# alibaba/animate-anything

Measured on AMD Instinct MI355X. Metric: UNet3D denoising steps/sec @16fx512x512 bs=1, higher is better.
Workload: dtype fp16; 1 GPU; animate_anything_512_v1.02 UNet3D (1413M params, seeded random init), 16 frames x 512x512, pipeline bs=1 per GPU (CFG batch 2, 17 frames inside), DPM-Solver++ step, hipGraph=on; clips_per_gpu=1, clips=1, parallelism=clip-sharded x1, collective=none

## Files before the change

### animate_anything_amd/_lib.py

```python
from __future__ import annotations

import ctypes as C
import os

import torch

AA_F16, AA_BF16, AA_F32 = 0, 1, 2
AA_ACT_NONE, AA_ACT_SILU, AA_ACT_GELU, AA_ACT_QUICK_GELU = 0, 1, 2, 3


class AaConvGemm(C.Structure):
    _fields_ = [
        ("a0", C.c_void_p), ("a1", C.c_void_p), ("w", C.c_void_p), ("bias", C.c_void_p),
        ("rowvec", C.c_void_p), ("residual", C.c_void_p), ("out", C.c_void_p),
        ("c0", C.c_int32), ("c1", C.c_int32),
        ("n_img", C.c_int32), ("h_in", C.c_int32), ("w_in", C.c_int32), ("h_virt", C.c_int32),
        ("w_virt", C.c_int32), ("h_out", C.c_int32), ("w_out", C.c_int32),
        ("kh", C.c_int32), ("kw", C.c_int32), ("stride", C.c_int32), ("pad_h", C.c_int32), ("pad_w", C.c_int32),
        ("n_out", C.c_int32), ("n_pad", C.c_int32), ("k_pad", C.c_int32),
        ("rowvec_div", C.c_int32), ("ldo", C.c_int32), ("ldr", C.c_int32),
        ("act", C.c_int32), ("geglu", C.c_int32), ("bias_per_row", C.c_int32),
        ("dtype", C.c_int32), ("out_dtype", C.c_int32), ("out_scale", C.c_float), ("workspace", C.c_void_p), ("workspace_bytes", C.c_int64), ("k_order", C.c_int32), ("debug", C.c_int32), ("tile", C.c_int32), ("k_splits", C.c_int32), ("rowvec_ld", C.c_int32), ("acc_scale", C.c_float),
        ("out_sy", C.c_int32), ("out_sx", C.c_int32), ("out_oy", C.c_int32), ("out_ox", C.c_int32),
        ("ln_stats", C.c_void_p), ("ln_cols", C.c_void_p), ("ln_parts", C.c_int32), ("ln_eps", C.c_float),
# ... 145 lines not shown

class AaFreeU(C.Structure):
    _fields_ = [
        ("hidden", C.c_void_p), ("hidden_out", C.c_void_p), ("skip", C.c_void_p), ("skip_out", C.c_void_p), ("trig", C.c_void_p),
        ("images", C.c_int32), ("h", C.c_int32), ("w", C.c_int32), ("c_hidden", C.c_int32), ("c_skip", C.c_int32),
        ("hidden_ld", C.c_int32), ("hidden_out_ld", C.c_int32), ("skip_ld", C.c_int32), ("skip_out_ld", C.c_int32),
        ("b", C.c_float), ("s", C.c_float), ("dtype", C.c_int32),
    ]


class AaCfgRescale(C.Structure):
    _fields_ = [
        ("tokens", C.c_void_p), ("out", C.c_void_p), ("factor", C.c_void_p),
        ("clips", C.c_int32), ("channels", C.c_int32), ("frames", C.c_int32), ("hw", C.c_int32), ("ld", C.c_int32), ("out_ld", C.c_int32),
        ("guidance", C.c_float), ("rescale", C.c_float), ("dtype", C.c_int32),
    ]


AA_WINDOW_MAX = 64


class AaWindow(C.Structure):
    _fields_ = [
        ("window_frames", C.c_int32), ("frame", C.c_int32 * AA_WINDOW_MAX), ("weight", C.c_float * AA_WINDOW_MAX),
        ("first", C.c_int32 * AA_WINDOW_MAX), ("last", C.c_int32 * AA_WINDOW_MAX),
    ]


class AaWindowGather(C.Structure):
    _fields_ = [
        ("src", C.c_void_p), ("dst", C.c_void_p),
        ("clips", C.c_int32), ("channels", C.c_int32), ("total_frames", C.c_int32), ("hw", C.c_int32),
        ("window", AaWindow),
    ]


class AaWindowMerge(C.Structure):
    _fields_ = [
        ("tokens", C.c_void_p), ("acc", C.c_void_p), ("merged", C.c_void_p),
        ("clips", C.c_int32), ("channels", C.c_int32), ("total_frames", C.c_int32), ("hw", C.c_int32), ("ld", C.c_int32), ("out_ld", C.c_int32),
        ("guidance_on", C.c_int32), ("guidance", C.c_float), ("dtype", C.c_int32),
        ("window", AaWindow),
    ]


class AaFreeInit(C.Structure):
    _fields_ = [
        ("x", C.c_void_p), ("n0", C.c_void_p), ("z", C.c_void_p), ("out", C.c_void_p), ("mask", C.c_void_p), ("twiddle", C.c_void_p),
        ("volumes", C.c_int32), ("frames", C.c_int32), ("h", C.c_int32), ("w", C.c_int32),
        ("a", C.c_float), ("s", C.c_float),
    ]


_I, _I32, _I64, _F, _V, _Z, _P = C.c_int, C.c_int32, C.c_int64, C.c_float, C.c_void_p, C.c_size_t, C.POINTER


def _launch(desc):
    return _I, [_P(desc), _V]


PROTOTYPES = {
    "aa_version": (_I, []),
    "aa_last_error": (C.c_char_p, []),
    "aa_conv_gemm_workspace": (_Z, [_P(AaConvGemm)]),
    "aa_conv_gemm": _launch(AaConvGemm),
    "aa_conv_gemm_group": (_I, [_P(_P(AaConvGemm)), _I32, _V]),
    "aa_conv_gemm_group_ok": (_I, [_P(_P(AaConvGemm)), _I32, _I32]),
    "aa_conv_gemm_launch_count": (_I, [_P(AaConvGemm)]),
    "aa_conv_gemm_tickets": (_I, [_P(AaConvGemm)]),
    "aa_conv_gemm_reduce_launches": (_I, [_P(AaConvGemm)]),
    "aa_conv_gemm_row_stats_parts": (_I, [_P(AaConvGemm)]),
    "aa_conv_gemm_row_coef_ok": (_I, [_P(AaConvGemm)]),
    "aa_ln_finalize": (_I, [_V, _I32, _V, _I64, _I32, _F, _V]),
    "aa_conv_gemm_tile_info": (_I, [_I, _P(_I32)]),
    "aa_conv_gemm_tile_flags": (_I, [_I]),
    "aa_conv_gemm_tile_ok": (_I, [_P(AaConvGemm), _I]),
    "aa_set_tile_override": (None, [_I]),
    "aa_groupnorm_workspace": (_Z, [_P(AaGroupNorm)]),
    "aa_set_groupnorm_two_pass": (None, [_I]),
    "aa_groupnorm_plan": (_I, [_P(AaGroupNorm), _P(_I32)]),
    "aa_groupnorm": (_I, [_P(AaGroupNorm), _V, _Z, _V]),
    "aa_groupnorm_coef": (_I, [_P(AaGroupNorm), _V, _Z, _V, _V]),
    "aa_layernorm": (_I, [_V, _V, _V, _V, _I64, _I32, _F, _I32, _V]),
    "aa_attention": _launch(AaAttention),
    "aa_seq_self_attention_ok": (_I, [_P(AaSeqSelfAttn)]),
    "aa_seq_self_attention": _launch(AaSeqSelfAttn),
    "aa_ff_fused_ok": (_I, [_P(AaFFFused)]),
    "aa_ff_fused": _launch(AaFFFused),
    "aa_linear_rows_ok": (_I, [_P(AaLinearRows)]),
    "aa_linear_rows": _launch(AaLinearRows),
    "aa_quant_rows_fp8": _launch(AaQuantRowsFp8),
    "aa_linear_fp8": _launch(AaLinearFp8),
    "aa_softmax_rows": (_I, [_V, _V, _I64, _I32, _I32, _I32, _I32, _V]),
    "aa_cfg_dpm_step": _launch(AaDpmStep),
    "aa_timestep_embedding": (_I, [_V, _V, _I32, _I32, _I32, _V]),
    "aa_pack_latents": _launch(AaPackLatents),
    "aa_cfg_dpm_step_tokens": _launch(AaDpmStepTok),
    "aa_blend": _launch(AaBlend),
    "aa_pack_frames": _launch(AaPackFrames),
    "aa_cfg_euler_step_tokens": _launch(AaEulerStepTok),
    "aa_cfg_ddim_step_tokens": _launch(AaDdimStepTok),
    "aa_cfg_unipc_step_tokens": _launch(AaUnipcStepTok),
    "aa_freeu_tokens": _launch(AaFreeU),
    "aa_cfg_rescale_workspace": (_Z, [_P(AaCfgRescale)]),
    "aa_cfg_rescale_tokens": (_I, [_P(AaCfgRescale), _V, _Z, _V]),
    "aa_window_gather_latents": _launch(AaWindowGather),
    "aa_window_merge_tokens": _launch(AaWindowMerge),
    "aa_freeinit_workspace": (_Z, [_P(AaFreeInit)]),
    "aa_freeinit_mix": (_I, [_P(AaFreeInit), _V, _Z, _V]),
}
SYMBOLS = tuple(PROTOTYPES)

DEFAULT_PATH = os.path.join(os.path.dirname(os.path.abspath(__file__)), "libaa_mi355.so")


def bind(path: str) -> C.CDLL:
    if not os.path.exists(path):
        raise RuntimeError(f"{path} is missing: build it with `python -m animate_anything_amd.build` "
                           "(hipcc --offload-arch=gfx950); this package has no fallback backend")
    lib = C.CDLL(path)
    for name, (restype, argtypes) in PROTOTYPES.items():
        if not hasattr(lib, name):
            raise RuntimeError(f"{path} does not export {name}")
        fn = getattr(lib, name)
        fn.restype, fn.argtypes = restype, argtypes
    return lib


_lib = None
_host_pointers_ok = False


def get() -> C.CDLL:
    global _lib
    if _lib is None:
        _lib = bind(os.environ.get("AA_LIBRARY") or DEFAULT_PATH)
    return _lib


def host_pointers_ok() -> bool:
    return _host_pointers_ok


class use_library:

    def __init__(self, lib, host_pointers=False):
        self.lib, self.host = lib, host_pointers

    def __enter__(self):
        global _lib, _host_pointers_ok
        self.prev = (_lib, _host_pointers_ok)
        _lib, _host_pointers_ok = self.lib, self.host
        return self.lib

    def __exit__(self, *a):
        global _lib, _host_pointers_ok
        _lib, _host_pointers_ok = self.prev
```

### animate_anything_amd/build.py

```python
import os
import subprocess

PKG = os.path.dirname(os.path.abspath(__file__))
ROOT = os.path.dirname(PKG)
CSRC = os.path.join(PKG, "csrc")
LIB = os.path.join(PKG, "libaa_mi355.so")


def _deps():
    deps = [os.path.join(ROOT, "include", "aa_mi355.h")]
    for d, _, fs in os.walk(CSRC):
        deps += [os.path.join(d, f) for f in fs if f.endswith((".h", ".hip"))]
    return deps


def source_id():
    import hashlib
    h = hashlib.sha256()
    for d in sorted(_deps()):
        h.update(os.path.relpath(d, ROOT).encode())
        h.update(open(d, "rb").read())
    return h.hexdigest()[:16]


PROBE_LIB = os.path.join(PKG, "libaa_mi355_probe.so")
TU_GROUPS = 8


def build(force=False, verbose=False, probe=False, ablate=0, variant=None):
    LIB = PROBE_LIB if probe else globals()["LIB"]
    if ablate:
        LIB = os.path.join(PKG, f"libaa_mi355_abl{ablate}.so")
    if variant:
        LIB = os.path.join(PKG, f"libaa_mi355_{variant[0]}.so")
    if not force and os.path.exists(LIB) and all(os.path.getmtime(LIB) >= os.path.getmtime(d) for d in _deps()):
        return LIB
    hipcc = os.environ.get("HIPCC", "/opt/rocm/bin/hipcc")
    flags = ["--offload-arch=gfx950", "-O3", "-std=c++17", "-fPIC", "-ffast-math", f"-DAA_TU_GROUPS={TU_GROUPS}",
             "-I", os.path.join(CSRC, "kernels", "device"), "-I", os.path.join(CSRC, "kernels"), "-I", CSRC,
             "-I", os.path.join(ROOT, "include")]
    if probe:
        flags.insert(0, "-DAA_PHASE_PROBE")
    if ablate:
        flags.insert(0, f"-DAA_X_ABLATE={int(ablate)}")
    if variant:
        flags = list(variant[1]) + flags
    if verbose:
        flags.insert(0, "-Rpass-analysis=kernel-resource-usage")
    obj_dir = os.path.join(PKG, "build", os.path.basename(LIB)[:-3])
    os.makedirs(obj_dir, exist_ok=True)
    jobs = [([os.path.join(CSRC, "aa_api.hip")], os.path.join(obj_dir, "aa_api.o"))]
    jobs += [([f"-DAA_TU_GROUP={g}", os.path.join(CSRC, "aa_tiles.hip")], os.path.join(obj_dir, f"aa_tiles_{g}.o")) for g in range(TU_GROUPS)]

    import hashlib
    api_only = {"attention.h", "seq_attention.h", "norm.h", "glue.h", "freeu.h", "cfg_rescale.h", "window.h", "freeinit.h", "ff_fused.h", "linear_rows.h", "linear_fp8.h"}

    def dep_hash(job):
        src, _ = job
        h = hashlib.sha256(repr((flags, [x for x in src if x.startswith("-D")])).encode())
        tiles = any("aa_tiles.hip" in x for x in src)
        for d in sorted(_deps()):
            if tiles and (os.path.basename(d) in api_only or d.endswith("aa_api.hip")):
                continue
            if not tiles and d.endswith("aa_tiles.hip"):
                continue
            h.update(d.encode())
            h.update(open(d, "rb").read())
        return h.hexdigest()

    def compile_one(job):
        src, obj = job
        key, stamp = dep_hash(job), obj + ".dephash"
        if not force and os.path.exists(obj) and os.path.exists(stamp) and open(stamp).read() == key:
            return obj
        subprocess.check_call([hipcc] + flags + ["-c"] + src + ["-o", obj])
        with open(stamp, "w") as f:
            f.write(key)
        return obj

    from concurrent.futures import ThreadPoolExecutor
    with ThreadPoolExecutor(max_workers=max(1, min(len(jobs), os.cpu_count() or 1))) as pool:
        objs = list(pool.map(compile_one, jobs))
    subprocess.check_call([hipcc, "--offload-arch=gfx950", "-shared", "-fPIC"] + objs + ["-o", LIB])
    import shutil
    have_tools = shutil.which(os.path.join(LLVM_TOOLS, "llvm-objdump")) and shutil.which(os.path.join(LLVM_TOOLS, "llvm-readelf"))
    if not ablate and os.environ.get("AA_BUILD_AUDIT", "1") != "0" and not have_tools:
        import json
        with open(LIB[:-3] + ".buildinfo.json", "w") as f:
            json.dump({"flags": flags, "audit": "skipped: llvm-objdump / llvm-readelf not found under " + LLVM_TOOLS}, f, indent=1)
    elif not ablate and os.environ.get("AA_BUILD_AUDIT", "1") != "0":
        problems = audit_x_kernels(LIB)
        info = {"hipcc": subprocess.run([hipcc, "--version"], capture_output=True, text=True).stdout.strip().split("\n"),
                "flags": flags, "audit": "ok" if not problems else problems}
        import json
        with open(LIB[:-3] + ".buildinfo.json", "w") as f:
            json.dump(info, f, indent=1)
        if problems:
            os.replace(LIB, LIB + ".rejected")
            raise RuntimeError("libaa_mi355.so: the code-object audit of the hand-scheduled kernels failed (library moved to "
                               + LIB + ".rejected):\n  " + "\n  ".join(str(p_) for p_ in problems[:8]))
    return LIB


LLVM_TOOLS = "/opt/rocm/lib/llvm/bin"


def device_code_objects(lib_path, out_dir):
    import struct
# ... 146 lines not shown
```

### animate_anything_amd/csrc/aa_api_impl.h

```cpp
#pragma once
#include <stdarg.h>
#include <stdio.h>
#include <stdlib.h>
#include <string.h>
#include "aa_mi355.h"
#include "kernels/conv_gemm.h"
#include "kernels/conv_gemm_dma.h"
#include "kernels/conv_slab.h"
#include "kernels/conv_gemm_x.h"
#include "kernels/norm.h"
#include "kernels/attention.h"
#include "kernels/seq_attention.h"
#include "kernels/ff_fused.h"
#include "kernels/linear_rows.h"
#include "kernels/linear_fp8.h"
#include "kernels/glue.h"
#include "kernels/freeu.h"
#include "kernels/cfg_rescale.h"
#include "kernels/window.h"
#include "kernels/freeinit.h"

namespace aa {

static thread_local char g_err[512] = "";

static int fail(int code, const char* fmt, ...) {
    va_list ap;
    va_start(ap, fmt);
    vsnprintf(g_err, sizeof(g_err), fmt, ap);
    va_end(ap);
    return code;
}

static int finish(const char* what) {
    const char* e = AA_POST_LAUNCH();
    if (e) return fail(AA_E_HIP, "%s: %s", what, e);
    return AA_OK;
}

static bool aligned_to(const void* p, uintptr_t bytes) { return (reinterpret_cast<uintptr_t>(p) & (bytes - 1)) == 0; }
static bool aligned16(const void* p) { return aligned_to(p, 16); }

template <typename T> struct DType16 { using type = T; };
template <typename F>
static bool with_dtype16(int dtype, F&& f) {
    if (dtype == AA_F16) { f(DType16<f16_t>{}); return true; }
    if (dtype == AA_BF16) { f(DType16<bf16_t>{}); return true; }
    return false;
}

template <typename D>
static bool step_tok_geometry_ok(const D* d, int ld) {
    return d->clips > 0 && d->channels > 0 && d->frames > 0 && d->hw > 0 && ld >= d->channels && d->next_t_count >= 0 && d->next_t_count <= 256;
}

template <typename D>
static dim3 step_tok_grid(const D* d) {
    const int64_t blocks = ((int64_t)d->clips * d->channels * d->frames * d->hw + 255) / 256;
    return dim3((unsigned)(blocks > 2048 ? 2048 : blocks));
}

struct CgCfg { int bm, bn, wm, wn, bk, stages, per_cu; float rate; int slab = 0; int x = 0; int sched = 0; };
constexpr int cg_dp(int dp3, int dp0, int dp1) { return (dp3 | dp0 << 4 | dp1 << 8) << 6; }
static const CgCfg kCgCfgs[] = {
    {128, 64, 2, 2, 64, 2, 3, 0.78f},
    {128, 128, 2, 2, 64, 2, 2, 0.90f},
    {192, 256, 3, 2, 64, 2, 1, 1.05f},
    {256, 256, 4, 2, 64, 2, 1, 1.10f},
    {256, 320, 4, 2, 64, 2, 1, 1.10f},
    {192, 320, 3, 2, 64, 2, 1, 1.05f},
    {256, 320, 4, 2, 32, 4, 1, 1.15f},
    {256, 256, 4, 2, 32, 4, 1, 1.15f},
    {128, 128, 2, 2, 32, 4, 2, 0.95f},
// ... 1222 lines not shown
    const dim3 grid((unsigned)((d->hw + WIN_THREADS - 1) / WIN_THREADS), (unsigned)d->window.window_frames, (unsigned)d->clips), block(WIN_THREADS);
    with_dtype16(d->dtype, [&](auto t) {
        using T = typename decltype(t)::type;
        if (vec) AA_LAUNCH((window_merge_kernel<T, true>), grid, block, 0, stream, *d);
        else AA_LAUNCH((window_merge_kernel<T, false>), grid, block, 0, stream, *d);
    });
    return finish("window_merge_tokens");
}

static bool freeinit_geometry_ok(const AaFreeInit* d) {
    if (d->volumes < 1 || d->frames < 1 || d->h < 1 || d->w < 1 || d->frames > aa::FI_MAX || d->h > aa::FI_MAX || d->w > aa::FI_MAX) return false;
    return (int64_t)d->volumes * d->frames * d->h * d->w < ((int64_t)1 << 31);
}

size_t aa_freeinit_workspace(const AaFreeInit* d) {
    if (!d || !freeinit_geometry_ok(d)) return 0;
    return (size_t)d->volumes * d->frames * d->h * d->w * 2 * sizeof(float);
}

int aa_freeinit_mix(const AaFreeInit* d, void* workspace, size_t workspace_bytes, void* stream) {
    using namespace aa;
    if (!d || !d->x || !d->n0 || !d->z || !d->out || !d->mask || !d->twiddle) return fail(AA_E_SHAPE, "freeinit_mix: null operand");
    if (!freeinit_geometry_ok(d))
        return fail(AA_E_SHAPE, "freeinit_mix: bad geometry (volumes %d, frames %d, h %d, w %d; every axis 1 .. %d)", d->volumes, d->frames, d->h,
                    d->w, FI_MAX);
    if (!finite_f32(&d->a) || !finite_f32(&d->s)) return fail(AA_E_SHAPE, "freeinit_mix: a and s must be finite");
    const size_t need = aa_freeinit_workspace(d);
    if (!workspace || workspace_bytes < need) return fail(AA_E_WORKSPACE, "freeinit_mix: workspace %zu < %zu bytes", workspace_bytes, need);
    if (!aligned_to(d->x, 4) || !aligned_to(d->n0, 4) || !aligned_to(d->z, 4) || !aligned_to(d->out, 4) || !aligned_to(d->mask, 4) ||
        !aligned_to(d->twiddle, 8) || !aligned_to(workspace, 8))
        return fail(AA_E_ALIGN, "freeinit_mix: x / n0 / z / out / mask must be 4-byte, the table and the workspace 8-byte aligned");
    const int64_t vol = (int64_t)d->frames * d->h * d->w, n = vol * d->volumes;
    const Span out = {d->out, n * 4}, ws = {workspace, (int64_t)need};
    const Span in[5] = {{d->x, n * 4}, {d->n0, n * 4}, {d->z, n * 4}, {d->mask, vol * 4}, {d->twiddle, (int64_t)(d->frames + d->h + d->w) * 8}};
    if (spans_overlap(out, in[0]) && d->out != d->x) return fail(AA_E_SHAPE, "freeinit_mix: out may be x itself or a separate buffer, not overlap it");
    for (int i = 1; i < 5; ++i)
        if (spans_overlap(out, in[i])) return fail(AA_E_SHAPE, "freeinit_mix: out must not overlap n0, z, the mask or the table");
    if (spans_overlap(out, ws)) return fail(AA_E_SHAPE, "freeinit_mix: the workspace must not overlap out");
    for (int i = 0; i < 5; ++i)
        if (spans_overlap(ws, in[i])) return fail(AA_E_SHAPE, "freeinit_mix: the workspace must not overlap an operand");
    f32x2* spec = (f32x2*)workspace;
    const f32x2* tw = (const f32x2*)d->twiddle;
    const dim3 block(FI_THREADS), rows((unsigned)fi_row_groups(*d));
    AA_LAUNCH(freeinit_rows_fwd_kernel<>, rows, block, FI_ROWS_FWD_LDS, stream, *d, spec);
    AA_LAUNCH((freeinit_axis_kernel<false>), dim3((unsigned)fi_axis_groups((int64_t)d->volumes * d->frames, d->w)), block, FI_AXIS_LDS, stream, spec,
              tw + fi_tw_h(*d), d->h, d->w);
    AA_LAUNCH(freeinit_frames_kernel<>, dim3((unsigned)fi_axis_groups(d->volumes, (int64_t)d->h * d->w)), block, FI_FRAMES_LDS, stream, *d, spec);
    AA_LAUNCH((freeinit_axis_kernel<true>), dim3((unsigned)fi_axis_groups((int64_t)d->volumes * d->frames, d->w)), block, FI_AXIS_LDS, stream, spec,
              tw + fi_tw_h(*d), d->h, d->w);
    AA_LAUNCH(freeinit_rows_inv_kernel<>, rows, block, FI_ROWS_INV_LDS, stream, *d, (const f32x2*)spec);
    return finish("freeinit_mix");
}

}
#endif
```

### animate_anything_amd/ops.py

```python
from __future__ import annotations

import ctypes as C
import math
import os
from dataclasses import dataclass
from typing import Optional

import torch

from . import _lib
from ._lib import (AA_ACT_GELU, AA_ACT_NONE, AA_ACT_QUICK_GELU, AA_ACT_SILU, AA_BF16, AA_F16, AA_F32, AaAttention, AaAttnOperand,
                   AaBlend, AaConvGemm, AaFFFused, AaLinearRows, AaLinearFp8, AaQuantRowsFp8, AaDdimStepTok, AaDpmStep, AaDpmStepTok, AaEulerStepTok, AaGroupNorm, AaPackFrames, AaPackLatents, AaSeqSelfAttn, AaUnipcStepTok, AaFreeU, AaCfgRescale, AaWindow, AaWindowGather, AaWindowMerge, AaFreeInit)

_DT = {torch.float16: AA_F16, torch.bfloat16: AA_BF16, torch.float32: AA_F32}

TRACE = None

AUTOTUNE = True
LAST_STAMPS = None
GN_PLANS = None
MAX_OPERAND_BYTES = 1 << 31
FORCE_TILE = -1
ATTN_FLAGS = int(os.environ.get("AA_ATTN_FLAGS", "0"))
if ATTN_FLAGS & ~13:
    raise RuntimeError(f"AA_ATTN_FLAGS={ATTN_FLAGS}: only bits 0 (value 1), 2 (value 4) and 3 (value 8) exist")
LN_FINALIZE_LAUNCH = os.environ.get("AA_LN_RAW", "0") != "1"
TILE_PICKER = None
PRODUCER_COEF = os.environ.get("AA_PRODUCER_COEF", "1") == "1"
LN_RAW_ANY_PARTS = False
K_SPLITS = 0
USE_TICKETS = os.environ.get("AA_TICKETS", "0") == "1"
DEBUG_ABLATE = int(os.environ.get("AA_DEBUG_ABLATE", "0"))
class _TileTable:

    def __init__(self):
        self._rows = None

    def _load(self):
        if self._rows is None:
            lib, rows, info = _lib.get(), [], (C.c_int32 * 7)()
            while lib.aa_conv_gemm_tile_info(len(rows), info) == 0:
                rows.append(tuple(info) + (int(lib.aa_conv_gemm_tile_flags(len(rows))),))
            self._rows = rows
        return self._rows

    def __iter__(self):
        return iter([(r[0], r[1], r[4], r[5]) for r in self._load()])

    def __len__(self):
        return len(self._load())

    def __getitem__(self, i):
        r = self._load()[i]
        return (r[0], r[1], r[4], r[5])

    def wave_cols(self, i):
        return self._load()[i][3]

    def per_cu(self, i):
        return self._load()[i][6]

    def flags(self, i):
        return self._load()[i][7]


# ... 631 lines not shown
def groupnorm(x0: torch.Tensor, gamma: torch.Tensor, beta: torch.Tensor, n_groups_img: int,
              tokens_per_group: int, num_groups: int = 32, eps: float = 1e-5, silu: bool = False,
              x1: Optional[torch.Tensor] = None, out: Optional[torch.Tensor] = None) -> torch.Tensor:
    lib = _lib.get()
    _check(x0, x1, gamma, beta, out)
    c0 = x0.shape[-1]
    c1 = 0 if x1 is None else x1.shape[-1]
    y = torch.empty(n_groups_img * tokens_per_group, c0 + c1, dtype=x0.dtype, device=x0.device) if out is None else out
    d = AaGroupNorm()
    d.x0, d.x1, d.gamma, d.beta, d.y = _ptr(x0), _ptr(x1), _ptr(gamma), _ptr(beta), _ptr(y)
    d.c0, d.c1 = c0, c1
    d.n_groups_img, d.tokens_per_group, d.num_groups = n_groups_img, tokens_per_group, num_groups
    d.silu, d.dtype, d.eps = int(silu), _DT[x0.dtype], eps
    nbytes = lib.aa_groupnorm_workspace(C.byref(d))
    ws = torch.empty(max(nbytes // 4, 1), dtype=torch.float32, device=x0.device)
    two_pass = False
    if AUTOTUNE and x0.is_cuda:
        key = (-1, d.dtype, c0, c1, n_groups_img, tokens_per_group, num_groups, int(silu))
        _load_default_tile_cache()
        choice = _tile_cache.get(key)
        if choice is None and y.data_ptr() != x0.data_ptr() and not torch.cuda.is_current_stream_capturing():
            choice = _autotune_groupnorm(lib, d, ws, nbytes, _stream(x0), key)
        two_pass = bool(choice and choice[0])
    if two_pass:
        lib.aa_set_groupnorm_two_pass(1)
    try:
        if GN_PLANS is not None:
            info = (C.c_int32 * 4)()
            GN_PLANS.append(tuple(info) if lib.aa_groupnorm_plan(C.byref(d), info) else None)
        _run(lib.aa_groupnorm, C.byref(d), _ptr(ws), nbytes, _stream(x0))
    finally:
        if two_pass:
            lib.aa_set_groupnorm_two_pass(0)
    return y


def groupnorm_coef(x0: torch.Tensor, gamma: torch.Tensor, beta: torch.Tensor, n_groups_img: int, tokens_per_group: int, num_groups: int = 32,
                   eps: float = 1e-5) -> torch.Tensor:
    lib = _lib.get()
    _check(x0, gamma, beta)
    c0 = x0.shape[-1]
    d = AaGroupNorm()
    d.x0, d.x1, d.gamma, d.beta, d.y = _ptr(x0), None, _ptr(gamma), _ptr(beta), None
    d.c0, d.c1 = c0, 0
    d.n_groups_img, d.tokens_per_group, d.num_groups = n_groups_img, tokens_per_group, num_groups
    d.silu, d.dtype, d.eps = 0, _DT[x0.dtype], eps
    nbytes = lib.aa_groupnorm_workspace(C.byref(d))
    ws = torch.empty(max(nbytes // 4, 1), dtype=torch.float32, device=x0.device)
    coef = torch.empty(n_groups_img, 2, c0, dtype=torch.float32, device=x0.device)
    _run(lib.aa_groupnorm_coef, C.byref(d), _ptr(ws), nbytes, _ptr(coef), _stream(x0))
    return coef


def layernorm(x: torch.Tensor, gamma: torch.Tensor, beta: torch.Tensor, eps: float = 1e-5) -> torch.Tensor:
    lib = _lib.get()
    _check(x, gamma, beta)
    y = torch.empty_like(x)
    _run(lib.aa_layernorm, _ptr(x), _ptr(gamma), _ptr(beta), _ptr(y), x.shape[0], x.shape[1], eps,
         _DT[x.dtype], _stream(x))
    return y


def _operand(t: torch.Tensor, col0: int, outer_stride: int, inner_stride: int, pos_stride: int, outer_div: int = 1):
    o = AaAttnOperand()
    o.ptr, o.ld, o.col0 = _ptr(t), t.stride(0), col0
    o.outer_stride, o.inner_stride, o.pos_stride, o.outer_div = outer_stride, inner_stride, pos_stride, outer_div
    return o


def attention(q: torch.Tensor, q_col0: int, k: torch.Tensor, k_col0: int, v: torch.Tensor, v_col0: int,
              heads: int, n_outer: int, n_inner: int, q_len: int, kv_len: int,
              q_strides, kv_strides, kv_outer_div: int = 1, scale: Optional[float] = None, head_dim: int = 64,
              kv_seq_mod: int = 0, causal: bool = False) -> torch.Tensor:
    lib = _lib.get()
    for t in (q, k, v):
        if not _addressable(t) or t.stride(-1) != 1:
            raise RuntimeError("attention: operands must be GPU tensors with contiguous rows")
    out = torch.empty(q.shape[0], heads * head_dim, dtype=q.dtype, device=q.device)
    d = AaAttention()
    d.q = _operand(q, q_col0, *q_strides)
    d.k = _operand(k, k_col0, *kv_strides, outer_div=kv_outer_div)
    d.v = _operand(v, v_col0, *kv_strides, outer_div=kv_outer_div)
    d.o = _operand(out, 0, *q_strides)
    d.k.seq_mod = d.v.seq_mod = kv_seq_mod
    d.causal = int(causal)
    d._pad = ATTN_FLAGS
    d.n_outer, d.n_inner, d.heads, d.head_dim = n_outer, n_inner, heads, head_dim
    d.q_len, d.kv_len, d.dtype = q_len, kv_len, _DT[q.dtype]
    d.scale = float(head_dim) ** -0.5 if scale is None else scale
    _run(lib.aa_attention, C.byref(d), _stream(q))
    return out


SEQ_ATTN_DEBUG = 0


@dataclass
class SeqQKV:
    w: torch.Tensor
    bias: Optional[torch.Tensor]
    ln_eps: float


def pack_seq_qkv(wq: torch.Tensor, wk: torch.Tensor, wv: torch.Tensor, ln=None) -> SeqQKV:
    n, c = wq.shape
    assert n % 64 == 0 and wk.shape == (n, c) and wv.shape == (n, c)
# ... 691 lines not shown
```

### animate_anything_amd/unet3d.py

```python
from __future__ import annotations

from dataclasses import dataclass
from types import SimpleNamespace
from typing import Optional

import torch
import torch.nn as nn

from . import ops
from ._model import GraphModel, Session
from .layers import (Attention, Conv2d, Downsample2D, Grid, GroupNorm, Linear, ResnetBlock2D, TemporalConvLayer,
                     TimestepEmbedding, Transformer2DModel, TransformerTemporalModel, Upsample2D)


@dataclass
class UNet3DConditionOutput:
    sample: torch.Tensor


class _Stage(nn.Module):

    def __init__(self, res_io, temb_channels, eps, groups, heads=None, head_dim=None, cross_attention_dim=None,
                 down=None, up=False):
        super().__init__()
# ... 176 lines not shown
            if kind not in _UP:
                raise ValueError(f"{kind} does not exist.")
            prev_c, out_c = out_c, rev[i]
            skip_c = rev[min(i + 1, n - 1)]
            L = layers_per_block + 1
            io = [((prev_c if j == 0 else out_c) + (skip_c if j == L - 1 else out_c), out_c) for j in range(L)]
            up = i < n - 1
            self.num_upsamplers += int(up)
            attn = dict(heads=out_c // rhd[i], head_dim=rhd[i], cross_attention_dim=cross_attention_dim) \
                if kind.startswith("CrossAttn") else {}
            self.up_blocks.append(_UP[kind](io, temb, norm_eps, norm_num_groups, up=up, **attn))
            self.up_blocks[-1].resolution_idx = i

        self.conv_norm_out = GroupNorm(norm_num_groups, ch0, eps=norm_eps)
        self.conv_act = nn.SiLU()
        self.conv_out = Conv2d(ch0, out_channels, 3, padding=1)
        self._graph = None
        from . import layers as _layers
        if _layers.AA_FP8_FF:
            self.enable_fp8_feedforward()

    def _project_text(self, text_tokens):
        self._project_batched(text_tokens, "_text_pack", lambda m: isinstance(m, Attention) and m.is_cross,
                              lambda a: (a.to_k, a.to_v), "kv")

    def _project_time_embeddings(self, temb_silu):
        self._project_batched(temb_silu, "_temb_pack", lambda m: isinstance(m, ResnetBlock2D) and m.time_emb_proj is not None,
                              lambda b: (b.time_emb_proj,), "tproj")

    def enable_gradient_checkpointing(self):
        self.gradient_checkpointing = True

    def disable_gradient_checkpointing(self):
        self.gradient_checkpointing = False

    def enable_xformers_memory_efficient_attention(self, *a, **k):
        return None

    def set_attention_slice(self, slice_size):
        return None

    def _core(self, sample, cond, mask, t, motion_t, cond_emb, text_tokens, g: Grid, text_len: int, upsample_sizes, cfg_dup=False):
        dt = text_tokens.dtype
        ch0 = self.conv_in.out_channels
        t_sin = ops.timestep_embedding(t, ch0, dt)
        cond_sin = ops.timestep_embedding(motion_t, ch0, dt) if motion_t is not None else cond_emb
        dup = 2 if (cfg_dup and g.clips % 2 == 0 and self.down_blocks[0].has_cross_attention) else 1
        g0 = Grid(g.clips // dup, g.frames, g.h, g.w)
        x8 = ops.pack_latents(sample, cond, mask, g0.clips, dt)
        temb_silu = self.time_embedding.tokens(t_sin, cond_sin, final_silu=True)
        self._project_time_embeddings(temb_silu)
        self._project_text(text_tokens)
        conv_in = self.conv_in2 if mask is not None else self.conv_in
        x = conv_in.tokens(x8, ops.conv3x3_geom(g0.images, g0.h, g0.w))
        if g.frames > 1:
            x = self.transformer_in.tokens(x, g0)
        skips = [(torch.cat([x] * dup) if dup > 1 else x, g)]
        for i, blk in enumerate(self.down_blocks):
            if i == 0:
                x, _, outs = blk.tokens(x, g0, temb_silu, text_tokens, text_len, dup=dup)
            else:
                x, g, outs = blk.tokens(x, g, temb_silu, text_tokens, text_len)
            if i == 0:
                g = outs[-1][1]
            skips += outs
        x = self.mid_block.tokens(x, g, temb_silu, text_tokens, text_len)
        for i, blk in enumerate(self.up_blocks):
            x, g = blk.tokens(x, g, skips, temb_silu, text_tokens, text_len, upsample_size=upsample_sizes[i])
        x = self.conv_norm_out.tokens(x, g.images, g.hw, silu=True)
        return ops.conv_gemm(x, self._conv_out_pack(), ops.conv3x3_geom(g.images, g.h, g.w))

    def _conv_out_pack(self):
        from .layers import weights_key
        w, b = self.conv_out.weight, self.conv_out.bias
        n = w.shape[0]
        if n % 8 == 0 or w.shape[1] % 64:
            return self.conv_out.packed()
        key = weights_key(w, b)
        if getattr(self, "_co_pack", None) is None or self._co_key != key:
            pad = (-n) % 8
            wp = torch.cat([w.detach(), torch.zeros((pad,) + tuple(w.shape[1:]), dtype=w.dtype, device=w.device)])
            bp = None if b is None else torch.cat([b.detach(), torch.zeros(pad, dtype=b.dtype, device=b.device)])
            self._co_pack, self._co_key = ops.pack_weight(wp, bp), key
        return self._co_pack

    def forward(self, sample, timestep, encoder_hidden_states, condition_latent, mask, class_labels=None,
                timestep_cond=None, attention_mask=None, cross_attention_kwargs=None,
                down_block_additional_residuals=None, mid_block_additional_residual=None, motion=None,
                return_dict=True, image_embeds=None):
        if down_block_additional_residuals is not None or mid_block_additional_residual is not None:
            raise NotImplementedError("ControlNet residual hooks are not part of the MI355X hot path")
        self.require_device(sample)
        dt, dev = self.dtype, sample.device
        b, _, frames, h, w = sample.shape
        t = timestep
        if not torch.is_tensor(t):
            t = torch.tensor([float(t)], dtype=torch.float32, device=dev)
        t = t.to(device=dev, dtype=torch.float32).reshape(-1).expand(b).contiguous()
        motion_t = cond_emb = None
        if self.motion_strength and motion is not None:
            motion_t = torch.as_tensor(motion, device=dev).to(torch.float32).reshape(-1).expand(b).contiguous()
        elif timestep_cond is not None:
            cond_emb = timestep_cond.to(dt).expand(b, self.conv_in.out_channels).contiguous()
        use_mask = bool(self.motion_mask and mask is not None)
        if sample.dtype not in (torch.float32, dt):
            sample = sample.to(dt)
        sess = self.session(b, frames, h, w, tuple(encoder_hidden_states.shape[1:]), use_mask, motion_t is not None,
                            cond_emb is not None, sample.dtype, sample.shape[0], condition_latent.shape[0],
                            mask.shape[0] if use_mask else 0, dev)
        sess.load(sample=sample, cond=condition_latent, mask=mask if use_mask else None, t=t, motion=motion_t,
                  cond_emb=cond_emb, text=encoder_hidden_states)
        y = sess.run()
        y = y.reshape(b, frames + 1, h, w, -1)[..., :self.conv_out.out_channels].permute(0, 4, 1, 2, 3)[:, :, 1:]
        return UNet3DConditionOutput(sample=y) if return_dict else (y,)

    def enable_fp8_feedforward(self, min_dim=None):
        from .layers import FP8_FF_MIN_DIM, FeedForward
        min_dim = FP8_FF_MIN_DIM if min_dim is None else min_dim
        n = 0
        for m in self.modules():
            if isinstance(m, FeedForward):
                m.fp8 = m.dim >= min_dim
                n += int(m.fp8)
# ... 59 lines not shown
```

### include/aa_mi355.h

```cpp
#ifndef AA_MI355_H
#define AA_MI355_H

#include <stddef.h>
#include <stdint.h>

#ifdef __cplusplus
extern "C" {
#endif

#define AA_VERSION 110

enum { AA_F16 = 0, AA_BF16 = 1, AA_F32 = 2 };
enum { AA_OK = 0, AA_E_SHAPE = -1, AA_E_DTYPE = -2, AA_E_ALIGN = -3, AA_E_WORKSPACE = -4, AA_E_HIP = -5 };
enum { AA_ACT_NONE = 0, AA_ACT_SILU = 1,
       AA_ACT_GELU = 2, AA_ACT_QUICK_GELU = 3  };

int aa_version(void);
const char* aa_last_error(void);

typedef struct AaConvGemm {
    const void* a0;
    const void* a1;
    const void* w;
    const void* bias;
// ... 364 lines not shown
    int32_t ld, out_ld;
    float guidance, rescale;
    int32_t dtype;
} AaCfgRescale;

size_t aa_cfg_rescale_workspace(const AaCfgRescale* d);
int aa_cfg_rescale_tokens(const AaCfgRescale* d, void* workspace, size_t workspace_bytes, void* stream);

#define AA_WINDOW_MAX 64
typedef struct AaWindow {
    int32_t window_frames;
    int32_t frame[AA_WINDOW_MAX];
    float weight[AA_WINDOW_MAX];
    int32_t first[AA_WINDOW_MAX];
    int32_t last[AA_WINDOW_MAX];
} AaWindow;

typedef struct AaWindowGather {
    const float* src;
    float* dst;
    int32_t clips, channels, total_frames, hw;
    AaWindow window;
} AaWindowGather;

typedef struct AaWindowMerge {
    const void* tokens;
    float* acc;
    void* merged;
    int32_t clips, channels, total_frames, hw;
    int32_t ld, out_ld;
    int32_t guidance_on;
    float guidance;
    int32_t dtype;
    AaWindow window;
} AaWindowMerge;

int aa_window_gather_latents(const AaWindowGather* d, void* stream);
int aa_window_merge_tokens(const AaWindowMerge* d, void* stream);

typedef struct AaFreeInit {
    const float* x;
    const float* n0;
    const float* z;
    float* out;
    const float* mask;
    const float* twiddle;
    int32_t volumes, frames, h, w;
    float a, s;
} AaFreeInit;

size_t aa_freeinit_workspace(const AaFreeInit* d);
int aa_freeinit_mix(const AaFreeInit* d, void* workspace, size_t workspace_bytes, void* stream);

#ifdef __cplusplus
}
#endif
#endif
```

Baseline: 16.82 steps/s.

## Add specialised thin-channel kernels for conv_in and fused norm+SiLU conv_out

Adds two dedicated kernels for the UNet's thin convolutions. One is a conv_in kernel for 8-channel inputs that keeps the weights in registers and issues direct MFMA over the 9 taps. The other is a conv_out kernel that applies the group-norm scale/shift and SiLU on the fly, computes per-tap partial products into LDS, and then sums the shifted taps into at most 8 output channels. This removes the separate normalized activation tensor write and read, and avoids running the general conv_gemm path on very thin N or K shapes. Both are gated by shape checks and an env flag, falling back to the old path otherwise.

```diff
diff --git a/animate_anything_amd/_lib.py b/animate_anything_amd/_lib.py
--- a/animate_anything_amd/_lib.py
+++ b/animate_anything_amd/_lib.py
@@ -221,7 +221,16 @@
     ]
 
 
-_I, _I32, _I64, _F, _V, _Z, _P = C.c_int, C.c_int32, C.c_int64, C.c_float, C.c_void_p, C.c_size_t, C.POINTER
+class AaConvThin(C.Structure):
+    _fields_ = [
+        ("x", C.c_void_p), ("w", C.c_void_p), ("bias", C.c_void_p), ("coef", C.c_void_p), ("out", C.c_void_p),
+        ("n_img", C.c_int32), ("h", C.c_int32), ("w_img", C.c_int32), ("channels", C.c_int32),
+        ("n_out", C.c_int32), ("n_pad", C.c_int32), ("k_pad", C.c_int32), ("k_order", C.c_int32),
+        ("ldx", C.c_int32), ("ldo", C.c_int32), ("dtype", C.c_int32), ("_pad", C.c_int32),
+    ]
+
+
+_I, _I32, _I64, _F, _V, _Z, _P =C.c_int, C.c_int32, C.c_int64, C.c_float, C.c_void_p, C.c_size_t, C.POINTER
 
 
 def _launch(desc):
@@ -277,6 +286,10 @@
     "aa_window_merge_tokens": _launch(AaWindowMerge),
     "aa_freeinit_workspace": (_Z, [_P(AaFreeInit)]),
     "aa_freeinit_mix": (_I, [_P(AaFreeInit), _V, _Z, _V]),
+    "aa_conv_in8_ok": (_I, [_P(AaConvThin)]),
+    "aa_conv_in8": _launch(AaConvThin),
+    "aa_conv_out_norm_ok": (_I, [_P(AaConvThin)]),
+    "aa_conv_out_norm": _launch(AaConvThin),
 }
 SYMBOLS = tuple(PROTOTYPES)
 
diff --git a/animate_anything_amd/build.py b/animate_anything_amd/build.py
--- a/animate_anything_amd/build.py
+++ b/animate_anything_amd/build.py
@@ -53,7 +53,7 @@
     jobs += [([f"-DAA_TU_GROUP={g}", os.path.join(CSRC, "aa_tiles.hip")], os.path.join(obj_dir, f"aa_tiles_{g}.o")) for g in range(TU_GROUPS)]
 
     import hashlib
-    api_only = {"attention.h", "seq_attention.h", "norm.h", "glue.h", "freeu.h", "cfg_rescale.h", "window.h", "freeinit.h", "ff_fused.h", "linear_rows.h", "linear_fp8.h"}
+    api_only = {"attention.h", "seq_attention.h", "norm.h", "glue.h", "freeu.h", "cfg_rescale.h", "window.h", "freeinit.h", "ff_fused.h", "linear_rows.h", "linear_fp8.h", "conv_thin.h"}
 
     def dep_hash(job):
         src, _ = job
diff --git a/animate_anything_amd/csrc/aa_api_impl.h b/animate_anything_amd/csrc/aa_api_impl.h
--- a/animate_anything_amd/csrc/aa_api_impl.h
+++ b/animate_anything_amd/csrc/aa_api_impl.h
@@ -19,6 +19,7 @@
 #include "kernels/cfg_rescale.h"
 #include "kernels/window.h"
 #include "kernels/freeinit.h"
+#include "kernels/conv_thin.h"
 
 namespace aa {
 
@@ -1347,5 +1348,51 @@
     return finish("freeinit_mix");
 }
 
+static bool conv_thin_common_ok(const AaConvThin* d) {
+    if (!d || (d->dtype != AA_F16 && d->dtype != AA_BF16)) return false;
+    if (d->n_img < 1 || d->h < 1 || d->w_img < 1 || d->channels < 8 || d->n_out < 1 || d->n_pad < d->n_out || d->k_pad % 8) return false;
+    if (d->ldx < d->channels || d->ldx % 8 || d->ldo % 8) return false;
+    const int64_t rows = (int64_t)d->n_img * d->h * d->w_img, lim = (int64_t)1 << 31;
+    return rows * d->ldx * 2 < lim && rows * d->ldo * 2 < lim;
+}
+
+int aa_conv_in8_ok(const AaConvThin* d) {
+    if (!conv_thin_common_ok(d)) return 0;
+    if (d->channels != 8 || d->ldx != 8 || d->k_order != 0 || d->k_pad < 80) return 0;
+    return d->n_out % 8 == 0 && d->n_pad % 64 == 0 && d->n_pad <= 512 && d->n_pad - d->n_out < 64 && d->ldo >= d->n_out;
+}
+
+int aa_conv_in8(const AaConvThin* d, void* stream) {
+    using namespace aa;
+    if (!aa_conv_in8_ok(d)) return fail(AA_E_SHAPE, "conv_in8: unsupported call (see aa_conv_in8_ok)");
+    if (!d->x || !d->w || !d->out) return fail(AA_E_SHAPE, "conv_in8: x, w, out are required");
+    if (!aligned16(d->x) || !aligned16(d->w) || !aligned16(d->out)) return fail(AA_E_ALIGN, "conv_in8: operands must be 16-byte aligned");
+    const int M = d->n_img * d->h * d->w_img, groups = (M + 31) / 32;
+    const dim3 grid((unsigned)(groups < 1024 ? groups : 1024)), block(d->n_pad);
+    with_dtype16(d->dtype, [&](auto t) { using T = typename decltype(t)::type; AA_LAUNCH((conv_in8_kernel<T>), grid, block, 0, stream, *d, M, groups); });
+    return finish("conv_in8");
+}
+
+int aa_conv_out_norm_ok(const AaConvThin* d) {
+    if (!conv_thin_common_ok(d)) return 0;
+    if (d->channels % 64 || d->n_out > 8 || d->ldo < 8) return 0;
+    if (d->k_pad < 9 * d->channels) return 0;
+    aa::CtoPlan pl;
+    return aa::cto_plan(*d, pl) ? 1 : 0;
+}
+
+int aa_conv_out_norm(const AaConvThin* d, void* stream) {
+    using namespace aa;
+    if (!aa_conv_out_norm_ok(d)) return fail(AA_E_SHAPE, "conv_out_norm: unsupported call (see aa_conv_out_norm_ok)");
+    if (!d->x || !d->w || !d->out || !d->coef) return fail(AA_E_SHAPE, "conv_out_norm: x, w, coef, out are required");
+    if (!aligned16(d->x) || !aligned16(d->w) || !aligned16(d->out) || !aligned16(d->coef)) return fail(AA_E_ALIGN, "conv_out_norm: operands must be 16-byte aligned");
+    CtoPlan pl;
+    cto_plan(*d, pl);
+    const int M = d->n_img * d->h * d->w_img;
+    const dim3 grid((unsigned)pl.blocks), block(CTO_THREADS);
+    with_dtype16(d->dtype, [&](auto t) { using T = typename decltype(t)::type; AA_LAUNCH((conv_out_norm_kernel<T>), grid, block, pl.lds, stream, *d, M, pl.bmg, pl.hg); });
+    return finish("conv_out_norm");
+}
+
 }
 #endif
diff --git a/animate_anything_amd/csrc/kernels/conv_thin.h b/animate_anything_amd/csrc/kernels/conv_thin.h
--- /dev/null
+++ b/animate_anything_amd/csrc/kernels/conv_thin.h
@@ -0,0 +1,198 @@
+#pragma once
+#include "dev.h"
+#include "aa_mi355.h"
+
+namespace aa {
+
+constexpr unsigned CT_OOB = 0x80000000u;
+
+__host__ __device__ inline int ct_row_pos(int i) { return 16 * ((i >> 2) & 1) + (i & 3) + 4 * (i >> 3); }
+
+template <typename T>
+__global__ void __launch_bounds__(512) conv_in8_kernel(const AaConvThin p, const int M, const int groups) {
+    const int lane = threadIdx.x & 63, wave = wave_id();
+    const int pcol = lane & 31, kh = lane >> 5;
+    const BufRsrc r_x = make_rsrc(p.x, (unsigned)M * 16u);
+    const BufRsrc r_out = make_rsrc(p.out, (unsigned)((int64_t)M * p.ldo * 2));
+    const T* w = reinterpret_cast<const T*>(p.w);
+    const T* bias = reinterpret_cast<const T*>(p.bias);
+
+    u32x4 wf[2][5];
+    f32x16 bv[2];
+#pragma unroll
+    for (int b = 0; b < 2; ++b) {
+        const T* row = w + (int64_t)(wave * 64 + b * 32 + ct_row_pos(pcol)) * p.k_pad;
+#pragma unroll
+        for (int s = 0; s < 5; ++s) wf[b][s] = *reinterpret_cast<const u32x4*>(row + (2 * s + kh) * 8);
+#pragma unroll
+        for (int e = 0; e < 16; ++e) {
+            const int n = wave * 64 + b * 32 + 16 * kh + e;
+            bv[b][e] = (bias && n < p.n_out) ? (float)bias[n] : 0.0f;
+        }
+    }
+    for (int g = blockIdx.x; g < groups; g += gridDim.x) {
+        const int m = g * 32 + pcol;
+        const int x = m % p.w_img, y = (m / p.w_img) % p.h;
+        u32x4 xf[5];
+#pragma unroll
+        for (int s = 0; s < 5; ++s) {
+            const int tap = 2 * s + kh, dy = tap / 3 - 1, dx = tap % 3 - 1;
+            const bool ok = m < M && tap < 9 && (unsigned)(y + dy) < (unsigned)p.h && (unsigned)(x + dx) < (unsigned)p.w_img;
+            xf[s] = buf_load16(r_x, ok ? (unsigned)(m + dy * p.w_img + dx) * 16u : CT_OOB);
+        }
+#pragma unroll
+        for (int b = 0; b < 2; ++b) {
+            f32x16 acc = bv[b];
+#pragma unroll
+            for (int s = 0; s < 5; ++s) acc = mfma_32x32x16(T(), wf[b][s], xf[s], acc);
+            const int n0 = wave * 64 + b * 32 + 16 * kh;
+#pragma unroll
+            for (int j = 0; j < 2; ++j) {
+                Pack8<T> o;
+#pragma unroll
+                for (int e = 0; e < 8; ++e) o.e[e] = (T)acc[8 * j + e];
+                const bool ok = m < M && n0 + 8 * j < p.n_out;
+                buf_store16(r_out, ok ? (unsigned)(((int64_t)m * p.ldo + n0 + 8 * j) * 2) : CT_OOB, o.raw);
+            }
+        }
+    }
+}
+
+constexpr int CTO_THREADS = 512;
+constexpr int CTO_LDS_MAX = 160 * 1024;
+
+struct CtoPlan { int bmg, hg, touch, blocks, lds; };
+
+__host__ __device__ inline int cto_quads(int n_out) { return (n_out + 3) / 4; }
+__host__ __device__ inline int cto_w_bytes(int channels) { return channels / 16 * 3 * 64 * 16; }
+__host__ __device__ inline int cto_p_bytes(int bmg, int hg, int n_out) { return (bmg + 2 * hg) * 32 * 9 * cto_quads(n_out) * 16; }
+
+inline bool cto_plan(const AaConvThin& d, CtoPlan& pl) {
+    const int64_t M = (int64_t)d.n_img * d.h * d.w_img;
+    const int groups = (int)((M + 31) / 32), hw = d.h * d.w_img;
+    pl.hg = (d.w_img + 1 + 31) / 32;
+    for (int rounds = 1; rounds <= 4096; ++rounds) {
+        const int bmg = (groups + 256 * rounds - 1) / (256 * rounds);
+        const int span = (bmg + 2 * pl.hg) * 32;
+        int touch = (span + hw - 2) / hw + 1;
+        if (touch > d.n_img) touch = d.n_img;
+        const int lds = cto_w_bytes(d.channels) + cto_p_bytes(bmg, pl.hg, d.n_out) + touch * 2 * d.channels * 4 + 32;
+        if (lds <= CTO_LDS_MAX) { pl.bmg = bmg; pl.touch = touch; pl.lds = lds; pl.blocks = (groups + bmg - 1) / bmg; return true; }
+        if (bmg == 1) break;
+    }
+    return false;
+}
+
+template <typename T>
+__global__ void __launch_bounds__(CTO_THREADS) conv_out_norm_kernel(const AaConvThin p, const int M, const int bmg, const int hg) {
+    const int C = p.channels, steps = C / 16, NQ = cto_quads(p.n_out), hw = p.h * p.w_img;
+    const int tid = threadIdx.x, lane = tid & 63, wave = wave_id();
+    const int pcol = lane & 31, kh = lane >> 5;
+    const int ng = bmg + 2 * hg;
+    const int m0 = blockIdx.x * bmg * 32, q0 = m0 - hg * 32, q_end = q0 + ng * 32;
+    char* lds = dyn_smem();
+    u32x4* sW = reinterpret_cast<u32x4*>(lds);
+    float* sP = reinterpret_cast<float*>(lds + cto_w_bytes(C));
+    float* sBias = sP + (size_t)ng * 32 * 9 * NQ * 4;
+    float* sCoef = sBias + 8;
+    const int img_lo = (q0 > 0 ? q0 : 0) / hw;
+    const int img_hi = ((q_end < M ? q_end : M) - 1) / hw;
+
+    const T* w = reinterpret_cast<const T*>(p.w);
+    for (int idx = tid; idx < steps * 3 * 64; idx += CTO_THREADS) {
+        const int l = idx & 63, b = (idx >> 6) % 3, s = idx / 192;
+        const int i = l & 31, tap = 4 * b + (i >> 3), n = i & 7, c = 16 * s + 8 * (l >> 5);
+        u32x4 v = {0u, 0u, 0u, 0u};
+        if (tap < 9 && n < p.n_out) {
+            const int k = p.k_order ? (c >> 6) * 576 + tap * 64 + (c & 63) : tap * C + c;
+            v = *reinterpret_cast<const u32x4*>(w + (int64_t)n * p.k_pad + k);
+        }
+        sW[idx] = v;
+    }
+    if (tid < 8) sBias[tid] = (p.bias && tid < p.n_out) ? (float)reinterpret_cast<const T*>(p.bias)[tid] : 0.0f;
+    for (int idx = tid; idx < (img_hi - img_lo + 1) * 2 * C; idx += CTO_THREADS) sCoef[idx] = p.coef[(int64_t)img_lo * 2 * C + idx];
+    __syncthreads();
+
+    const BufRsrc r_x = make_rsrc(p.x, (unsigned)((int64_t)M * p.ldx * 2));
+    constexpr int NWV = CTO_THREADS / 64;
+    const int nch = steps / 4, iters = (ng - wave + NWV - 1) / NWV * nch;
+    auto fetch = [&](u32x4 (&dst)[4], int it) {
+        const int q = q0 + 32 * (wave + NWV * (it / nch)) + pcol;
+        const unsigned o = (q >= 0 && q < M) ? (unsigned)(((int64_t)q * p.ldx + 8 * kh) * 2) : CT_OOB;
+#pragma unroll
+        for (int j = 0; j < 4; ++j) dst[j] = buf_load16(r_x, o + 128u * (it % nch) + 32u * j);
+    };
+    u32x4 cur[4], nxt[4];
+    f32x16 acc[3];
+    const float* coef = sCoef;
+    if (iters > 0) fetch(cur, 0);
+    for (int it = 0; it < iters; ++it) {
+        if (it + 1 < iters) fetch(nxt, it + 1);
+        const int g = wave + NWV * (it / nch), ch = it % nch;
+        if (ch == 0) {
+            const int q = q0 + 32 * g + pcol;
+            coef = sCoef + (size_t)((q >= 0 && q < M ? q / hw : img_lo) - img_lo) * 2 * C + 8 * kh;
+#pragma unroll
+            for (int b = 0; b < 3; ++b)
+#pragma unroll
+                for (int e = 0; e < 16; ++e) acc[b][e] = 0.0f;
+        }
+#pragma unroll
+        for (int j = 0; j < 4; ++j) {
+            const int s = 4 * ch + j;
+            Pack8<T> v, a;
+            v.raw = cur[j];
+            const f32x4 sc0 = *reinterpret_cast<const f32x4*>(coef + 16 * s), sc1 = *reinterpret_cast<const f32x4*>(coef + 16 * s + 4);
+            const f32x4 sh0 = *reinterpret_cast<const f32x4*>(coef + C + 16 * s), sh1 = *reinterpret_cast<const f32x4*>(coef + C + 16 * s + 4);
+#pragma unroll
+            for (int e = 0; e < 8; ++e) {
+                const float f = (float)v.e[e] * (e < 4 ? sc0[e & 3] : sc1[e & 3]) + (e < 4 ? sh0[e & 3] : sh1[e & 3]);
+                a.e[e] = (T)(f / (1.0f + __expf(-f)));
+            }
+#pragma unroll
+            for (int b = 0; b < 3; ++b) acc[b] = mfma_32x32x16(T(), sW[(s * 3 + b) * 64 + lane], a.raw, acc[b]);
+        }
+        if (ch == nch - 1 && kh < NQ) {
+            float* dst = sP + ((size_t)(32 * g + pcol) * 9 * NQ + kh) * 4;
+#pragma unroll
+            for (int b = 0; b < 3; ++b)
+#pragma unroll
+                for (int tl = 0; tl < 4; ++tl)
+                    if (4 * b + tl < 9)
+                        *reinterpret_cast<f32x4*>(dst + (size_t)(4 * b + tl) * NQ * 4) = f32x4{acc[b][4 * tl], acc[b][4 * tl + 1], acc[b][4 * tl + 2], acc[b][4 * tl + 3]};
+        }
+        if (it + 1 < iters) {
+#pragma unroll
+            for (int j = 0; j < 4; ++j) cur[j] = nxt[j];
+        }
+    }
+    __syncthreads();
+
+    T* out = reinterpret_cast<T*>(p.out);
+    for (int px = tid; px < bmg * 32; px += CTO_THREADS) {
+        const int m = m0 + px;
+        if (m >= M) continue;
+        const int x = m % p.w_img, y = (m / p.w_img) % p.h;
+        float o[8];
+#pragma unroll
+        for (int e = 0; e < 8; ++e) o[e] = sBias[e];
+        for (int tap = 0; tap < 9; ++tap) {
+            const int dy = tap / 3 - 1, dx = tap % 3 - 1;
+            if ((unsigned)(y + dy) >= (unsigned)p.h || (unsigned)(x + dx) >= (unsigned)p.w_img) continue;
+            const float* src = sP + ((size_t)(px + hg * 32 + dy * p.w_img + dx) * 9 + tap) * NQ * 4;
+#pragma unroll
+            for (int qd = 0; qd < 2; ++qd)
+                if (qd < NQ) {
+                    const f32x4 v = *reinterpret_cast<const f32x4*>(src + 4 * qd);
+#pragma unroll
+                    for (int e = 0; e < 4; ++e) o[4 * qd + e] += v[e];
+                }
+        }
+        Pack8<T> r;
+#pragma unroll
+        for (int e = 0; e < 8; ++e) r.e[e] = (T)o[e];
+        *reinterpret_cast<u32x4*>(out + (int64_t)m * p.ldo) = r.raw;
+    }
+}
+
+}
diff --git a/animate_anything_amd/ops.py b/animate_anything_amd/ops.py
--- a/animate_anything_amd/ops.py
+++ b/animate_anything_amd/ops.py
@@ -10,7 +10,7 @@
 
 from . import _lib
 from ._lib import (AA_ACT_GELU, AA_ACT_NONE, AA_ACT_QUICK_GELU, AA_ACT_SILU, AA_BF16, AA_F16, AA_F32, AaAttention, AaAttnOperand,
-                   AaBlend, AaConvGemm, AaFFFused, AaLinearRows, AaLinearFp8, AaQuantRowsFp8, AaDdimStepTok, AaDpmStep, AaDpmStepTok, AaEulerStepTok, AaGroupNorm, AaPackFrames, AaPackLatents, AaSeqSelfAttn, AaUnipcStepTok, AaFreeU, AaCfgRescale, AaWindow, AaWindowGather, AaWindowMerge, AaFreeInit)
+                   AaBlend, AaConvGemm, AaFFFused, AaLinearRows, AaLinearFp8, AaQuantRowsFp8, AaDdimStepTok, AaDpmStep, AaDpmStepTok, AaEulerStepTok, AaGroupNorm, AaPackFrames, AaPackLatents, AaSeqSelfAttn, AaUnipcStepTok, AaFreeU, AaCfgRescale, AaWindow, AaWindowGather, AaWindowMerge, AaFreeInit, AaConvThin)
 
 _DT = {torch.float16: AA_F16, torch.bfloat16: AA_BF16, torch.float32: AA_F32}
 
@@ -748,6 +748,67 @@
     return coef
 
 
+CONV_THIN = os.environ.get("AA_CONV_THIN", "1") == "1"
+
+
+def _conv_thin_desc(x, pw: PackedWeight, g: Geom, n_out: int, out, coef=None) -> AaConvThin:
+    d = AaConvThin()
+    d.x, d.w, d.bias, d.coef, d.out = _ptr(x), _ptr(pw.w), _ptr(pw.bias), _ptr(coef), _ptr(out)
+    d.n_img, d.h, d.w_img = g.n_img, g.h_in, g.w_in
+    d.channels, d.n_out, d.n_pad, d.k_pad, d.k_order = x.shape[-1], n_out, pw.n_pad, pw.k_pad, pw.k_order
+    d.ldx, d.ldo = x.stride(0), 0 if out is None else out.stride(0)
+    d.dtype = _DT.get(x.dtype, -1)
+    return d
+
+
+def _conv_thin_geom_ok(x, pw: PackedWeight, g: Geom) -> bool:
+    return (pw.kh == 3 and pw.kw == 3 and g.stride == 1 and g.pad_h == 1 and g.pad_w == 1 and (g.h_out, g.w_out) == (g.h_in, g.w_in)
+            and (g.h_virt or g.h_in, g.w_virt or g.w_in) == (g.h_in, g.w_in) and x.dim() == 2 and x.shape[0] == g.rows
+            and x.shape[1] == pw.cin and pw.geglu == 0 and pw.ln_cols is None and x.dtype == pw.w.dtype)
+
+
+def conv_in8_ok(x: torch.Tensor, pw: PackedWeight, g: Geom) -> bool:
+    if not (CONV_THIN and _conv_thin_geom_ok(x, pw, g)):
+        return False
+    d = _conv_thin_desc(x, pw, g, pw.n_out, None)
+    d.ldo = pw.n_out
+    return bool(_lib.get().aa_conv_in8_ok(C.byref(d)))
+
+
+def conv_in8(x: torch.Tensor, pw: PackedWeight, g: Geom, out: Optional[torch.Tensor] = None) -> torch.Tensor:
+    if not _conv_thin_geom_ok(x, pw, g):
+        raise RuntimeError("conv_in8: a 3x3 / stride 1 / pad 1 convolution of a [rows, 8] token matrix with weights packed for it")
+    if out is None:
+        out = torch.empty(g.rows, pw.n_out, dtype=x.dtype, device=x.device)
+    _check(x, pw.w, pw.bias)
+    _check_token_matrix("conv_in8", "out", out, x, "both", device_of=("x", x), rows=g.rows, channels=pw.n_out)
+    d = _conv_thin_desc(x, pw, g, pw.n_out, out)
+    _run(_lib.get().aa_conv_in8, C.byref(d), _stream(x))
+    return out
+
+
+def conv_out_norm_ok(x: torch.Tensor, pw: PackedWeight, g: Geom, n_out: int) -> bool:
+    if not (CONV_THIN and _conv_thin_geom_ok(x, pw, g) and 1 <= n_out <= min(8, pw.n_out)):
+        return False
+    d = _conv_thin_desc(x, pw, g, n_out, None)
+    d.ldo = 8
+    return bool(_lib.get().aa_conv_out_norm_ok(C.byref(d)))
+
+
+def conv_out_norm(x: torch.Tensor, coef: torch.Tensor, pw: PackedWeight, g: Geom, n_out: int, out: Optional[torch.Tensor] = None) -> torch.Tensor:
+    if not (_conv_thin_geom_ok(x, pw, g) and 1 <= n_out <= min(8, pw.n_out) and coef.dtype == torch.float32 and coef.is_contiguous()
+            and tuple(coef.shape) == (g.n_img, 2, x.shape[1])):
+        raise RuntimeError("conv_out_norm: a 3x3 / stride 1 / pad 1 convolution to at most 8 channels with fp32 [images, 2, C] coefficients")
+    if out is None:
+        out = torch.empty(g.rows, 8, dtype=x.dtype, device=x.device)
+    _check(pw.w, pw.bias, coef)
+    _check_token_matrix("conv_out_norm", "x", x, x, "both")
+    _check_token_matrix("conv_out_norm", "out", out, x, "both", device_of=("x", x), rows=g.rows, channels=8)
+    d = _conv_thin_desc(x, pw, g, n_out, out, coef)
+    _run(_lib.get().aa_conv_out_norm, C.byref(d), _stream(x))
+    return out
+
+
 def layernorm(x: torch.Tensor, gamma: torch.Tensor, beta: torch.Tensor, eps: float = 1e-5) -> torch.Tensor:
     lib = _lib.get()
     _check(x, gamma, beta)
diff --git a/animate_anything_amd/unet3d.py b/animate_anything_amd/unet3d.py
--- a/animate_anything_amd/unet3d.py
+++ b/animate_anything_amd/unet3d.py
@@ -252,7 +252,11 @@
         self._project_time_embeddings(temb_silu)
         self._project_text(text_tokens)
         conv_in = self.conv_in2 if mask is not None else self.conv_in
-        x = conv_in.tokens(x8, ops.conv3x3_geom(g0.images, g0.h, g0.w))
+        geom_in = ops.conv3x3_geom(g0.images, g0.h, g0.w)
+        if ops.conv_in8_ok(x8, conv_in.packed(), geom_in):
+            x = ops.conv_in8(x8, conv_in.packed(), geom_in)
+        else:
+            x = conv_in.tokens(x8, geom_in)
         if g.frames > 1:
             x = self.transformer_in.tokens(x, g0)
         skips = [(torch.cat([x] * dup) if dup > 1 else x, g)]
@@ -267,8 +271,12 @@
         x = self.mid_block.tokens(x, g, temb_silu, text_tokens, text_len)
         for i, blk in enumerate(self.up_blocks):
             x, g = blk.tokens(x, g, skips, temb_silu, text_tokens, text_len, upsample_size=upsample_sizes[i])
+        geom_out, pw_out = ops.conv3x3_geom(g.images, g.h, g.w), self._conv_out_pack()
+        if pw_out.n_out == 8 and ops.conv_out_norm_ok(x, pw_out, geom_out, self.conv_out.out_channels):
+            coef = self.conv_norm_out.coef_tokens(x, g.images, g.hw)
+            return ops.conv_out_norm(x, coef, pw_out, geom_out, self.conv_out.out_channels)
         x = self.conv_norm_out.tokens(x, g.images, g.hw, silu=True)
-        return ops.conv_gemm(x, self._conv_out_pack(), ops.conv3x3_geom(g.images, g.h, g.w))
+        return ops.conv_gemm(x, pw_out, geom_out)
 
     def _conv_out_pack(self):
         from .layers import weights_key
diff --git a/include/aa_mi355.h b/include/aa_mi355.h
--- a/include/aa_mi355.h
+++ b/include/aa_mi355.h
@@ -440,6 +440,25 @@
 size_t aa_freeinit_workspace(const AaFreeInit* d);
 int aa_freeinit_mix(const AaFreeInit* d, void* workspace, size_t workspace_bytes, void* stream);
 
+typedef struct AaConvThin {
+    const void* x;
+    const void* w;
+    const void* bias;
+    const float* coef;
+    void* out;
+    int32_t n_img, h, w_img;
+    int32_t channels;
+    int32_t n_out, n_pad, k_pad, k_order;
+    int32_t ldx, ldo;
+    int32_t dtype;
+    int32_t _pad;
+} AaConvThin;
+
+int aa_conv_in8_ok(const AaConvThin* d);
+int aa_conv_in8(const AaConvThin* d, void* stream);
+int aa_conv_out_norm_ok(const AaConvThin* d);
+int aa_conv_out_norm(const AaConvThin* d, void* stream);
+
 #ifdef __cplusplus
 }
 #endif
```

After: 16.87 steps/s, median of 6. No clear change (+0.3%).
